# Geunwoo-Jeon/LarvaNet

Hardware: AMD Instinct MI355X
Metric: HR Mpixels/s (LarvaNet x4 multi-exit train step, 48x48 LR patches) (higher is better)
Workload: dtype f32; 1 GPU; LarvaNet x4 train_step_larva M4 B4,4,4,4 48ch, batch 16 of 3x48x48 -> 3x192x192 fp32 per GPU (BASELINE config 2); global_batch=16, parallelism=dp1, hip_graph=True

## Files before the change

larvanet_amd/csrc/conv3x3_mfma.hip:

```cpp
#include "larva_common.h"
#include "larva_bicubic.h"
#include <hip/hip_ext.h>
#include <cstdlib>
#include <type_traits>

#ifndef LARVA_DIAG
#define LARVA_DIAG 0
#endif
constexpr int kWgPerCu = 2;
constexpr int kOperandDepth = 2;


#ifndef LARVA_DIAG_ONLY48
#define LARVA_DIAG_ONLY48 0
#endif

namespace larva {

#if defined(LARVA_DIAG) && (LARVA_DIAG & 32)
__device__ unsigned long long* g_stamps = nullptr;
#if LARVA_DIAG & 512
constexpr int kDiagWgPerSlot = 256;
__device__ int g_slot_of_launch = 0;
__device__ __forceinline__ void stamp_slot(unsigned long long* area, int k) {
// ... 89 lines not shown
  static constexpr int CS = cout_stride(COUT);
  static constexpr int PS = G::PS;
  static constexpr int IN_PIECES = (kCh * PS + 255) / 256;
  static constexpr int IN_FLOATS = IN_PIECES * 256;
  static constexpr int IN_SLOTS_PER_PLANE = PS / 4;
  static constexpr int W_USED = 9 * kCh * CS;
  static constexpr int W_PIECES = (W_USED + 255) / 256;
  static constexpr int W_FLOATS = W_PIECES * 256;
  static constexpr int PIECES = IN_PIECES + W_PIECES;
  static constexpr int NPW = (PIECES + 3) / 4;
  static constexpr int STAGE_FLOATS = IN_FLOATS + W_FLOATS;
  static constexpr int STEPS = 9 * (kCh / 4);
  static constexpr int NST = 3;
  static constexpr int AHEAD = NST - 1;
  static constexpr size_t LDS_BYTES_DMA = NST * STAGE_FLOATS * sizeof(float);
  static constexpr bool LOADER = 2 * PIECES <= 63;
  static constexpr int THREADS_DMA = LOADER ? 320 : 256;
  static constexpr size_t LDS_BYTES_REG = 2 * STAGE_FLOATS * sizeof(float);
  static constexpr int RIN_SLOTS = kCh * G::HALO * (G::RS / 4);
  static constexpr int RIN_ITERS = (RIN_SLOTS + 255) / 256;
  static constexpr int RW_SLOTS = W_USED / 4;
  static constexpr int RW_ITERS = (RW_SLOTS + 255) / 256;
  static_assert(kCh * PS <= IN_FLOATS, "input planes must fit their pieces");
};

template <int COUT, typename G>
struct DmaPlan {
  unsigned voff[ConvCfg<COUT, G>::NPW];
};

template <int COUT, typename G, bool WEIGHTS>
__device__ __forceinline__ void make_plan(const ConvArgs& a, int wave, int lane, int y0, int x0,
                                          DmaPlan<COUT, G>& pl) {
  using C = ConvCfg<COUT, G>;
#pragma unroll
  for (int i = 0; i < C::NPW; ++i) {
    const int p = min(wave + 4 * i, C::PIECES - 1);
    const bool isw = p >= C::IN_PIECES;
    if constexpr (WEIGHTS) {
      if (4 * i + 3 < C::IN_PIECES) continue;
      const int ws = (p - C::IN_PIECES) * 64 + lane;
      if (isw) pl.voff[i] = (ws * 4 < C::W_USED) ? 16u * (unsigned)ws : kDmaZero;
    } else {
      if (4 * i >= C::IN_PIECES) continue;
      const int slot = p * 64 + lane;
      const int ci = slot / C::IN_SLOTS_PER_PLANE;
      const int rem = slot - ci * C::IN_SLOTS_PER_PLANE;
      const int r = rem / (G::RS / 4);
      const int q = rem - r * (G::RS / 4);
      const int gy = y0 - 1 + r, gx = x0 - 4 + 4 * q;
      const bool ok = ci < kCh && r < G::HALO && gy >= 0 && gy < a.H && gx >= 0 && gx < a.W;
      if (!isw) pl.voff[i] = ok ? 4u * (unsigned)((ci * a.H + gy) * a.pitch + gx) : kDmaZero;
    }
  }
}

struct ChunkSrc {
  i32x4 img;
  i32x4 wgt;
  const float* img_ptr;
  const float* wgt_ptr;
};

template <int COUT, typename G>
__device__ __forceinline__ ChunkSrc chunk_src(const ConvArgs& a, int chunk, int n, const float* src_override = nullptr) {
  using C = ConvCfg<COUT, G>;
  const int c0 = chunk * kCh;
  const int s_idx = div_by_magic(chunk, a.magic_cps);
  const int c_in_src = c0 - s_idx * a.cin_per_src;
  ChunkSrc cs;
  const float* src = src_override ? src_override : a.src[0];
  if (s_idx != 0) {
    asm volatile("" ::: "memory");
    src = a.src[s_idx];
  }
  cs.img_ptr = src + ((size_t)n * a.cin_per_src + c_in_src) * ((size_t)a.H * a.pitch);
  cs.wgt_ptr = a.wpk + (size_t)chunk * C::W_USED;
  cs.img = dma_rsrc(cs.img_ptr);
  cs.wgt = dma_rsrc(cs.wgt_ptr);
  return cs;
}

template <int COUT, typename G>
__device__ __forceinline__ void dma_piece(const DmaPlan<COUT, G>& pl, int i, int wave, const ChunkSrc& cs,
                                          unsigned stage_addr) {
  using C = ConvCfg<COUT, G>;
  const int p = min(wave + 4 * i, C::PIECES - 1);
  const bool isw = p >= C::IN_PIECES;
  i32x4 rsrc;
#pragma unroll
  for (int k = 0; k < 4; ++k) rsrc[k] = isw ? cs.wgt[k] : cs.img[k];
  lds_dma16_buf(rsrc, pl.voff[i], 0, stage_addr + 1024u * (unsigned)p);
}

template <int COUT, typename G>
struct LoaderPlan {
  unsigned voff[ConvCfg<COUT, G>::PIECES];
};

template <int COUT, typename G>
__device__ __forceinline__ void make_loader_plan(const ConvArgs& a, int lane, int y0, int x0, LoaderPlan<COUT, G>& pl) {
  using C = ConvCfg<COUT, G>;
#pragma unroll
  for (int p = 0; p < C::PIECES; ++p) {
    if (p < C::IN_PIECES) {
      const int slot = p * 64 + lane;
      const int ci = slot / C::IN_SLOTS_PER_PLANE;
      const int rem = slot - ci * C::IN_SLOTS_PER_PLANE;
      const int r = rem / (G::RS / 4);
      const int q = rem - r * (G::RS / 4);
      const int gy = y0 - 1 + r, gx = x0 - 4 + 4 * q;
      const bool ok = ci < kCh && r < G::HALO && gy >= 0 && gy < a.H && gx >= 0 && gx < a.W;
      pl.voff[p] = ok ? 4u * (unsigned)((ci * a.H + gy) * a.pitch + gx) : kDmaZero;
    } else {
      const int ws = (p - C::IN_PIECES) * 64 + lane;
      pl.voff[p] = (ws * 4 < C::W_USED) ? 16u * (unsigned)ws : kDmaZero;
    }
  }
}

template <int COUT, typename G>
__device__ __forceinline__ void run_loader(const ConvArgs& a, float* smem, int lane, int n, int y0, int x0) {
  using C = ConvCfg<COUT, G>;
  if constexpr ((LARVA_DIAG & 256) != 0) return;
  LoaderPlan<COUT, G> pl;
  make_loader_plan<COUT, G>(a, lane, y0, x0, pl);
  const int last = a.n_chunks - 1;
  int stage = 0;
  for (int chunk = 0; chunk <= last; ++chunk) {
    asm volatile("; LARVA_RING loader chunk_pieces=%1 ahead=%2\n\ts_waitcnt vmcnt(%0)\n\ts_barrier" ::"n"((C::AHEAD - 1) * C::PIECES), "n"(C::PIECES), "n"(C::AHEAD) : "memory");
    __builtin_amdgcn_sched_barrier(0);
    const int nstage = (stage + C::AHEAD) % C::NST;
    const unsigned dst = lds_addr_of(smem + nstage * C::STAGE_FLOATS);
    const ChunkSrc cs = chunk_src<COUT, G>(a, min(chunk + C::AHEAD, last), n);
#pragma unroll
    for (int p = 0; p < C::PIECES; ++p)
      lds_dma16_buf(p < C::IN_PIECES ? cs.img : cs.wgt, pl.voff[p], 0, dst + 1024u * (unsigned)p);
    stage = stage == C::NST - 1 ? 0 : stage + 1;
  }
  asm volatile("s_waitcnt vmcnt(0)" ::: "memory");
}

template <int COUT, typename G>
struct RegStaging {
  f32x4 in[ConvCfg<COUT, G>::RIN_ITERS];
  f32x4 w[ConvCfg<COUT, G>::RW_ITERS];
};

template <int COUT, typename G>
__device__ __forceinline__ void reg_load(const ConvArgs& a, const ChunkSrc& cs, int y0, int x0, int tid,
                                         RegStaging<COUT, G>& st) {
  using C = ConvCfg<COUT, G>;
  const size_t plane = (size_t)a.H * a.pitch;
#pragma unroll
  for (int i = 0; i < C::RIN_ITERS; ++i) {
    const int s = min(tid + i * 256, C::RIN_SLOTS - 1);
    const int ci = s / (G::HALO * (G::RS / 4));
    const int rem = s - ci * (G::HALO * (G::RS / 4));
    const int r = rem / (G::RS / 4);
    const int q = rem - r * (G::RS / 4);
    const int gy = y0 - 1 + r, gx = x0 - 4 + 4 * q;
    const bool row_ok = gy >= 0 && gy < a.H;
    const float* row = cs.img_ptr + (size_t)ci * plane + (size_t)min(max(gy, 0), a.H - 1) * a.pitch;
    f32x4 v;
#pragma unroll
    for (int e = 0; e < 4; ++e) {
// ... 35 lines not shown
template <int COUT, typename G, int NCT, int PG0, int NPG>
__device__ __forceinline__ void read_operands(const float* const (&a_base)[NCT], const float* b_base, int step,
                                              float (&av)[NCT], float (&bv)[NPG]) {
  using C = ConvCfg<COUT, G>;
  if constexpr ((LARVA_DIAG & 128) != 0) {
#pragma unroll
    for (int c = 0; c < NCT; ++c) av[c] = (float)step;
#pragma unroll
    for (int p = 0; p < NPG; ++p) bv[p] = (float)(step + p);
    return;
  }
  const int tap = step / (kCh / 4), kk = step % (kCh / 4);
  const int ky = tap / 3, kx = tap % 3;
#pragma unroll
  for (int c = 0; c < NCT; ++c) av[c] = a_base[c][(tap * kCh + kk * 4) * C::CS];
#pragma unroll
  for (int p = 0; p < NPG; ++p) {
    const int pg = PG0 + p, prow = pg / G::PC, pcol = pg % G::PC;
    bv[p] = b_base[kk * 4 * C::PS + (prow + ky) * G::RS + pcol * 16 + kx];
  }
}

template <int NMF, int NRD, int M>
__device__ __forceinline__ void shadow_groups() {
  if constexpr (M < NMF) {
    __builtin_amdgcn_sched_group_barrier(0x8, 1, 0);
    constexpr int share = (NRD + NMF - 1 - M) / NMF;
    if constexpr (share > 0) __builtin_amdgcn_sched_group_barrier(0x100, share, 0);
    shadow_groups<NMF, NRD, M + 1>();
  }
}

template <int COUT, typename G, int NCT, int PG0, int NPG, bool SWAP>
__device__ __forceinline__ void mfma_chunk(const float* stage, int ct0, int lane, f32x4 (&acc)[NCT][NPG],
                                           const float* wstage = nullptr) {
  using C = ConvCfg<COUT, G>;
  const int lr = lane & 15, lq = lane >> 4;
  const float* const wrows = wstage ? wstage : stage + C::IN_FLOATS;
  const float* a_base[NCT];
#pragma unroll
  for (int c = 0; c < NCT; ++c)
    a_base[c] = wrows + lq * C::CS + lr + (cout_swizzled(COUT) ? (((ct0 + c) ^ (lq & 1)) * 16) : (ct0 + c) * 16);
  const float* b_base = stage + lq * C::PS + lr + 3;
  constexpr int D = kOperandDepth;
  float av[D + 1][NCT], bv[D + 1][NPG];
#pragma unroll
  for (int d = 0; d < D; ++d)
    if (d < C::STEPS) read_operands<COUT, G, NCT, PG0, NPG>(a_base, b_base, d, av[d], bv[d]);
#pragma unroll
  for (int step = 0; step < C::STEPS; ++step) {
    __builtin_amdgcn_sched_barrier(0);
    if (step + D < C::STEPS)
      read_operands<COUT, G, NCT, PG0, NPG>(a_base, b_base, step + D, av[(step + D) % (D + 1)], bv[(step + D) % (D + 1)]);
    constexpr int NMF = NCT * NPG;
    constexpr int NRD = NCT + NPG;
#pragma unroll
    for (int m = 0; m < NMF; ++m) {
      const float wv = av[step % (D + 1)][m / NPG], xv = bv[step % (D + 1)][m % NPG];
      acc[m / NPG][m % NPG] = __builtin_amdgcn_mfma_f32_16x16x4f32(SWAP ? xv : wv, SWAP ? wv : xv, acc[m / NPG][m % NPG], 0, 0, 0);
    }
    shadow_groups<NMF, NRD, 0>();
    __builtin_amdgcn_sched_barrier(0);
  }
}

template <int KEEP, int PIECES, int AUX>
__device__ __forceinline__ void wait_and_barrier() {
  static_assert(KEEP == PIECES + AUX, "a ring wait keeps exactly the next chunk's pieces and the operand loads in flight");
  asm volatile("; LARVA_RING pieces=%1 aux=%2\n\ts_waitcnt vmcnt(%0)\n\ts_barrier" ::"n"(KEEP), "n"(PIECES), "n"(AUX) : "memory");
  __builtin_amdgcn_sched_barrier(0);
}

template <typename G>
__device__ __forceinline__ void decode_tile(const ConvArgs& a, int vb, int& n, int& y0, int& x0) {
  const int tile = xcd_remap(vb, a.nwg);
  const int t2 = div_by_magic(tile, a.magic_tx);
  const int tx = tile - t2 * a.tiles_x;
  n = div_by_magic(t2, a.magic_ty);
  const int ty = t2 - n * a.tiles_y;
  x0 = tx * G::COLS;
  y0 = ty * G::ROWS;
}

template <int COUT, typename G, bool VEC, int EPI, int NCT, int PG0, int NPG, bool PERSIST = false>
__device__ __forceinline__ void run_role(const ConvArgs& a, float* smem, int ct0, int wave, int n, int y0, int x0, int tid) {
  using C = ConvCfg<COUT, G>;
  static_assert(!VEC || C::LOADER, "the 16-byte path runs with a loader wave (2 * PIECES <= 63 for every instantiated shape)");
  static_assert(!PERSIST || VEC, "persistent tiles: the loader-wave path");
  const int lane = tid & 63;
  const int lr = lane & 15, lq = lane >> 4;
  float* const out_ptr = a.out;
  struct { int H, W, pitch, plain; } k = {a.H, a.W, a.pitch, a.plain_stores};
  asm volatile("" : "+s"(k.H), "+s"(k.W), "+s"(k.pitch), "+s"(k.plain));

  constexpr bool kShuffleEpi = (EPI == kEpiShuffle || EPI == kEpiShuffleBase || EPI == kEpiShuffleL1);
  constexpr bool kPixMajor = VEC && !kShuffleEpi;
  f32x4 bias[NCT];
#pragma unroll
  for (int c = 0; c < NCT; ++c) bias[c] = f32x4{0.f, 0.f, 0.f, 0.f};
  auto load_bias = [&]() {
    if (a.bias) {
#pragma unroll
      for (int c = 0; c < NCT; ++c)
#pragma unroll
        for (int r = 0; r < 4; ++r) bias[c][r] = a.bias[(ct0 + c) * 16 + (kPixMajor ? lr : lq * 4 + r)];
    }
  };

  constexpr int NAUX = (EPI == kEpiMask || EPI == kEpiRes1 || EPI == kEpiShuffleBase)
                           ? 1 : ((EPI == kEpiRes2 || EPI == kEpiShuffleL1) ? 2 : 0);
  f32x4 aux[NAUX > 0 ? NAUX : 1][NAUX > 0 ? NCT : 1][NAUX > 0 ? NPG : 1];
  constexpr int NU = NCT * NPG;
  constexpr int kEarlyPairs = PERSIST && COUT == 48 ? (NAUX * NU < 7 ? NAUX * NU : 7) : NAUX * NU;
  constexpr int kLatePart = 4, kEarlyAll = 5;
  auto load_aux = [&](int part = -1) {
#pragma unroll
    for (int c = 0; c < NCT; ++c)
#pragma unroll
      for (int p = 0; p < NPG; ++p) {
        const int pg = PG0 + p, prow = pg / G::PC, pcol = pg % G::PC;
        const int y = min(y0 + prow, a.H - 1), x = min(x0 + pcol * 16 + lr, a.W - 1);
        auto want = [&](int op) {
          const int q = op * NU + c * NPG + p;
          return part < 0 ? true : part == kLatePart ? q >= kEarlyPairs : q < kEarlyPairs;
        };
        if constexpr (kShuffleEpi) {
          const int HH = 4 * a.H, WW = 4 * a.W;
          const size_t idx = (((size_t)n * C::CT + (ct0 + c)) * HH + (4 * y + lq)) * WW + 4 * x;
          if (want(0)) aux[0][c][p] = *reinterpret_cast<const f32x4*>(a.base + idx);
          if constexpr (EPI == kEpiShuffleL1) {
            if (want(1)) aux[1][c][p] = *reinterpret_cast<const f32x4*>(a.truth + idx);
          }
        } else if constexpr (kPixMajor && (PERSIST || G::COLS == 16)) {
          const unsigned plane = (unsigned)a.H * (unsigned)a.pitch;
          const unsigned lane_off = 4u * ((unsigned)lr * plane + (unsigned)lq * 4u);
          const int soff = __builtin_amdgcn_readfirstlane(
              (int)(4u * ((unsigned)((ct0 + c) * 16) * plane + (unsigned)(y0 + prow) * (unsigned)a.pitch + (unsigned)(x0 + pcol * 16))));
          auto image = [&](const float* t) {
            const unsigned long long b = reinterpret_cast<unsigned long long>(t + (size_t)n * COUT * plane);
            const unsigned lo = (unsigned)__builtin_amdgcn_readfirstlane((int)(unsigned)b);
            const unsigned hi = (unsigned)__builtin_amdgcn_readfirstlane((int)(unsigned)(b >> 32));
            return __builtin_amdgcn_make_buffer_rsrc(reinterpret_cast<void*>(((unsigned long long)hi << 32) | lo), 0,
                                                     (int)(COUT * plane * 4u), 0x00020000);
          };
          if constexpr (EPI == kEpiMask) {
            if (want(0)) aux[0][c][p] = __builtin_bit_cast(f32x4, __builtin_amdgcn_raw_buffer_load_b128(image(a.mask), lane_off, soff, 0));
          }
          if constexpr (EPI == kEpiRes1 || EPI == kEpiRes2) {
            if (want(0)) aux[0][c][p] = __builtin_bit_cast(f32x4, __builtin_amdgcn_raw_buffer_load_b128(image(a.res0), lane_off, soff, 0));
          }
          if constexpr (EPI == kEpiRes2) {
            if (want(1)) aux[1][c][p] = __builtin_bit_cast(f32x4, __builtin_amdgcn_raw_buffer_load_b128(image(a.res1), lane_off, soff, 0));
          }
        } else if constexpr (kPixMajor) {
          const size_t plane = (size_t)a.H * a.pitch;
          const int xb = min(x0 + pcol * 16 + lq * 4, a.pitch - 4);
          const size_t idx = ((size_t)n * COUT + (ct0 + c) * 16 + lr) * plane + (size_t)y * a.pitch + xb;
          if constexpr (EPI == kEpiMask) {
            if (want(0)) aux[0][c][p] = *reinterpret_cast<const f32x4*>(a.mask + idx);
          }
          if constexpr (EPI == kEpiRes1 || EPI == kEpiRes2) {
            if (want(0)) aux[0][c][p] = *reinterpret_cast<const f32x4*>(a.res0 + idx);
          }
          if constexpr (EPI == kEpiRes2) {
            if (want(1)) aux[1][c][p] = *reinterpret_cast<const f32x4*>(a.res1 + idx);
          }
        } else {
          const size_t plane = (size_t)a.H * a.pitch;
          const size_t idx0 = ((size_t)n * COUT + (ct0 + c) * 16 + lq * 4) * plane + (size_t)y * a.pitch + x;
#pragma unroll
          for (int r = 0; r < 4; ++r) {
            if constexpr (EPI == kEpiMask) aux[0][c][p][r] = a.mask[idx0 + r * plane];
            if constexpr (EPI == kEpiRes1 || EPI == kEpiRes2) aux[0][c][p][r] = a.res0[idx0 + r * plane];
            if constexpr (EPI == kEpiRes2) aux[1][c][p][r] = a.res1[idx0 + r * plane];
          }
        }
      }
  };
  constexpr bool kAuxLate = VEC && !kShuffleEpi && !(LARVA_DIAG & 6) && NAUX > 0 && !PERSIST;
  constexpr int kAuxLoads = kAuxLate ? NAUX * NCT * NPG : 0;
  auto load_early = [&]() {
    load_bias();
    if constexpr (NAUX > 0 && !kAuxLate && !(LARVA_DIAG & 4)) load_aux();
  };
  int pstage = 0;
  for (int vb = blockIdx.x;; vb += gridDim.x) {
  if constexpr (PERSIST) {
    if (vb >= a.nwg) break;
    decode_tile<G>(a, vb, n, y0, x0);
  }
  if constexpr (!VEC || (LARVA_DIAG & 2)) load_early();

  f32x4 acc[NCT][NPG];
#pragma unroll
  for (int c = 0; c < NCT; ++c)
#pragma unroll
    for (int p = 0; p < NPG; ++p) acc[c][p] = f32x4{0.f, 0.f, 0.f, 0.f};

  if constexpr (PERSIST) {
    load_bias();
    const int my_chunk = a.n_chunks >= 4 ? (wave & 3) : 0;
    __builtin_amdgcn_sched_barrier(0);
    for (int chunk = 0; chunk < a.n_chunks; ++chunk) {
      asm volatile("s_barrier" ::: "memory");
      __builtin_amdgcn_sched_barrier(0);
      if constexpr (NAUX > 0) {
        if (chunk == my_chunk) load_aux(kEarlyAll);
        __builtin_amdgcn_sched_barrier(0);
      }
      mfma_chunk<COUT, G, NCT, PG0, NPG, kPixMajor>(smem + pstage * C::STAGE_FLOATS, ct0, lane, acc);
      pstage = pstage == C::NST - 1 ? 0 : pstage + 1;
    }
    asm volatile("s_waitcnt vmcnt(0)" ::: "memory");
    __builtin_amdgcn_sched_barrier(0);
    if constexpr (kEarlyPairs < NAUX * NU) {
      load_aux(kLatePart);
      __builtin_amdgcn_sched_barrier(0);
    }
  } else if constexpr (VEC) {
    DmaPlan<COUT, G> pl;
    const int last = a.n_chunks - 1;
    if constexpr (!(LARVA_DIAG & 2)) {
      const ChunkSrc cs0 = chunk_src<COUT, G>(a, 0, n);
      const unsigned st0 = lds_addr_of(smem), st1 = lds_addr_of(smem + C::STAGE_FLOATS);
      stamp(6);
      make_plan<COUT, G, true>(a, wave, lane, y0, x0, pl);
#pragma unroll
      for (int i = 0; i < C::NPW; ++i)
        if (wave + 4 * i >= C::IN_PIECES) dma_piece<COUT, G>(pl, i, wave, cs0, st0);
      __builtin_amdgcn_sched_barrier(0);
      stamp(7);
      load_early();
      stamp(14);
      make_plan<COUT, G, false>(a, wave, lane, y0, x0, pl);
#pragma unroll
      for (int i = 0; i < C::NPW; ++i)
        if (wave + 4 * i < C::IN_PIECES) dma_piece<COUT, G>(pl, i, wave, cs0, st0);
      stamp(15);
      const ChunkSrc cs1 = chunk_src<COUT, G>(a, min(1, last), n);
#pragma unroll
      for (int i = 0; i < C::NPW; ++i) dma_piece<COUT, G>(pl, i, wave, cs1, st1);
      if constexpr (kAuxLate) {
        __builtin_amdgcn_sched_barrier(0);
        load_aux();
        __builtin_amdgcn_sched_barrier(0);
      }
    }
    stamp(1);
    int stage = 0;
    for (int chunk = 0; chunk <= last; ++chunk) {
      if constexpr ((LARVA_DIAG & 256) != 0) {
      } else if (chunk == 0) wait_and_barrier<((LARVA_DIAG & 2) ? 0 : C::NPW) + kAuxLoads, ((LARVA_DIAG & 2) ? 0 : C::NPW), kAuxLoads>();
      else wait_and_barrier<kAuxLoads, 0, kAuxLoads>();
      if (chunk == 0) stamp(2);
      stamp(8 + (chunk < 7 ? chunk : 7));
      if constexpr (!(LARVA_DIAG & 1)) mfma_chunk<COUT, G, NCT, PG0, NPG, kPixMajor>(smem + stage * C::STAGE_FLOATS, ct0, lane, acc);
      stage = stage == C::NST - 1 ? 0 : stage + 1;
    }
    asm volatile("s_waitcnt vmcnt(0)" ::: "memory");
    stamp(3);
  } else {
    RegStaging<COUT, G> st;
    if constexpr (!(LARVA_DIAG & 2)) {
      reg_load<COUT, G>(a, chunk_src<COUT, G>(a, 0, n), y0, x0, tid, st);
      reg_store<COUT, G>(smem, tid, st);
    }
    __syncthreads();
    for (int chunk = 0; chunk < a.n_chunks; ++chunk) {
      float* cur = smem + (chunk & 1) * C::STAGE_FLOATS;
      float* nxt = smem + ((chunk & 1) ^ 1) * C::STAGE_FLOATS;
      const bool more = chunk + 1 < a.n_chunks;
      if constexpr (!(LARVA_DIAG & 2)) {
        if (more) reg_load<COUT, G>(a, chunk_src<COUT, G>(a, chunk + 1, n), y0, x0, tid, st);
      }
      if constexpr (!(LARVA_DIAG & 1)) mfma_chunk<COUT, G, NCT, PG0, NPG, kPixMajor>(cur, ct0, lane, acc);
      if constexpr (!(LARVA_DIAG & 2)) {
        if (more) reg_store<COUT, G>(nxt, tid, st);
      }
      __syncthreads();
    }
  }

  if constexpr ((LARVA_DIAG & 4) != 0) {
#pragma unroll
    for (int c = 0; c < NCT; ++c)
#pragma unroll
      for (int p = 0; p < NPG; ++p) asm volatile("" ::"v"(acc[c][p]));
    return;
  }

  if constexpr (EPI == kEpiShuffleL1) {
    const int HH = 4 * k.H, WW = 4 * k.W;
    const size_t plane = (size_t)k.H * k.pitch;
    const float g = a.gval;
    float s = 0.f;
#pragma unroll
    for (int c = 0; c < NCT; ++c)
#pragma unroll
      for (int p = 0; p < NPG; ++p) {
        const int pg = PG0 + p, prow = pg / G::PC, pcol = pg % G::PC;
        const int y = y0 + prow, x = x0 + pcol * 16 + lr;
        const f32x4 v = (acc[c][p] + bias[c]) + aux[0][c][p];
        if (y < k.H && x < k.W) {
          if (out_ptr) {
            const size_t idx = (((size_t)n * C::CT + (ct0 + c)) * HH + (4 * y + lq)) * WW + 4 * x;
            __builtin_nontemporal_store(v, reinterpret_cast<f32x4*>(out_ptr + idx));
          }
          const f32x4 d = v - aux[1][c][p];
          s += fabsf(d[0]) + fabsf(d[1]) + fabsf(d[2]) + fabsf(d[3]);
          const size_t idx0 = ((size_t)n * COUT + (ct0 + c) * 16 + lq * 4) * plane + (size_t)y * k.pitch + x;
#pragma unroll
          for (int r = 0; r < 4; ++r)
            __builtin_nontemporal_store(d[r] > 0.f ? g : (d[r] < 0.f ? -g : 0.f), &a.grad[idx0 + r * plane]);
        }
      }
#pragma unroll
    for (int o = 32; o > 0; o >>= 1) s += __shfl_xor(s, o);
    if (lane == 0) a.partial[4 * blockIdx.x + wave] = s;
  } else if constexpr (EPI == kEpiShuffle || EPI == kEpiShuffleBase) {
    const int HH = 4 * k.H, WW = 4 * k.W;
#pragma unroll
    for (int c = 0; c < NCT; ++c)
#pragma unroll
      for (int p = 0; p < NPG; ++p) {
        const int pg = PG0 + p, prow = pg / G::PC, pcol = pg % G::PC;
        const int y = y0 + prow, x = x0 + pcol * 16 + lr;
        const size_t idx = (((size_t)n * C::CT + (ct0 + c)) * HH + (4 * y + lq)) * WW + 4 * x;
        f32x4 v = acc[c][p] + bias[c];
        if constexpr (EPI == kEpiShuffleBase) v += aux[0][c][p];
        if (y < k.H && x < k.W) __builtin_nontemporal_store(v, reinterpret_cast<f32x4*>(out_ptr + idx));
      }
  } else if constexpr (kPixMajor) {
    const size_t plane = (size_t)k.H * k.pitch;
    auto store_all = [&](auto plain_tag, auto interior_tag) {
      constexpr bool kPlain = decltype(plain_tag)::value;
      constexpr bool kInterior = decltype(interior_tag)::value;
#pragma unroll
      for (int c = 0; c < NCT; ++c)
#pragma unroll
        for (int p = 0; p < NPG; ++p) {
          const int pg = PG0 + p, prow = pg / G::PC, pcol = pg % G::PC;
          const int y = y0 + prow, xb = x0 + pcol * 16 + lq * 4;
          const size_t idx = ((size_t)n * COUT + (ct0 + c) * 16 + lr) * plane + (size_t)y * k.pitch + xb;
          f32x4 v = acc[c][p] + bias[c];
          if (kInterior || (y < k.H && xb < k.pitch)) {
#pragma unroll
            for (int r = 0; r < 4; ++r) {
              float o = v[r];
              if constexpr (EPI == kEpiRelu) o = fmaxf(o, 0.f);
              if constexpr (EPI == kEpiMask) o = (aux[0][c][p][r] > 0.f) ? o : 0.f;
              if constexpr (EPI == kEpiRes1 || EPI == kEpiRes2) o += aux[0][c][p][r];
              if constexpr (EPI == kEpiRes2) o += aux[1][c][p][r];
              v[r] = (kInterior || xb + r < k.W) ? o : 0.f;
            }
            if constexpr (kPlain) *reinterpret_cast<f32x4*>(out_ptr + idx) = v;
            else __builtin_nontemporal_store(v, reinterpret_cast<f32x4*>(out_ptr + idx));
          }
        }
    };
    constexpr bool kFastPath = EPI == kEpiPlain || EPI == kEpiRelu || EPI == kEpiRes1;
    const bool interior = kFastPath && y0 + G::ROWS <= k.H && x0 + G::COLS <= k.W;
    auto store_policy = [&](auto plain_tag) {
      if constexpr (kFastPath) {
        if (interior) {
          store_all(plain_tag, std::true_type{});
          return;
        }
      }
      store_all(plain_tag, std::false_type{});
    };
    if constexpr ((LARVA_DIAG & 16) != 0) {
      store_policy(std::true_type{});
    } else if constexpr (G::COLS == 16) {
      if (k.plain) store_policy(std::true_type{});
      else store_policy(std::false_type{});
    } else {
      store_policy(std::false_type{});
    }
  } else {
    const size_t plane = (size_t)k.H * k.pitch;
#pragma unroll
    for (int c = 0; c < NCT; ++c)
#pragma unroll
      for (int p = 0; p < NPG; ++p) {
        const int pg = PG0 + p, prow = pg / G::PC, pcol = pg % G::PC;
        const int y = y0 + prow, x = x0 + pcol * 16 + lr;
        const size_t idx0 = ((size_t)n * COUT + (ct0 + c) * 16 + lq * 4) * plane + (size_t)y * k.pitch + x;
        const f32x4 v = acc[c][p] + bias[c];
        if (y < k.H && x < k.pitch) {
          const bool real = x < k.W;
#pragma unroll
          for (int r = 0; r < 4; ++r) {
            float o = v[r];
            if constexpr (EPI == kEpiRelu) o = fmaxf(o, 0.f);
            if constexpr (EPI == kEpiMask) o = (aux[0][c][p][r] > 0.f) ? o : 0.f;
            if constexpr (EPI == kEpiRes1 || EPI == kEpiRes2) o += aux[0][c][p][r];
            if constexpr (EPI == kEpiRes2) o += aux[1][c][p][r];
            o = real ? o : 0.f;
            if constexpr ((LARVA_DIAG & 16) != 0) out_ptr[idx0 + r * plane] = o;
            else __builtin_nontemporal_store(o, &out_ptr[idx0 + r * plane]);
          }
        }
      }
  }
#if LARVA_DIAG & 32
  stamp(4);
  asm volatile("s_waitcnt vmcnt(0)" ::: "memory");
  stamp(5);
#endif
  if constexpr (!PERSIST) break;
  }
}

__device__ __forceinline__ void fetch_args(const ConvArgs& a) {
  asm volatile("" ::"s"(a.src[0]), "s"(a.wpk), "s"(a.bias), "s"(a.out), "s"(a.cin_per_src), "s"(a.n_chunks), "s"(a.N),
               "s"(a.H), "s"(a.W), "s"(a.pitch), "s"(a.tiles_x), "s"(a.tiles_y), "s"(a.magic_tx), "s"(a.magic_ty),
               "s"(a.magic_cps), "s"(a.nwg), "s"(a.tile_tab), "s"(a.plain_stores), "s"(a.tab_n),
               "s"(a.tab16[0]), "s"(a.tab16[16]));
}

template <int COUT, bool VEC, int EPI, typename G = GeoWide>
__device__ __forceinline__ void conv_tile(const ConvArgs& a, float* smem) {
  if constexpr ((LARVA_DIAG & 8) != 0) return;
  stamp(0);
  fetch_args(a);
  const int tile = xcd_remap(blockIdx.x, a.nwg);
  const int t2 = div_by_magic(tile, a.magic_tx);
  const int tx = tile - t2 * a.tiles_x;
  const int n = div_by_magic(t2, a.magic_ty);
  const int ty = t2 - n * a.tiles_y;
  const int x0 = tx * G::COLS, y0 = ty * G::ROWS;
  const int tid = threadIdx.x;
  const int wave = __builtin_amdgcn_readfirstlane(tid >> 6);
  __builtin_amdgcn_s_setprio(1);

  if constexpr (VEC) {
    if (wave == 4) {
      if constexpr (!(LARVA_DIAG & 2)) run_loader<COUT, G>(a, smem, tid & 63, n, y0, x0);
      return;
    }
  }
  if constexpr (G::ROWS == 4) {
    static_assert(VEC && (COUT == 48 || COUT == 32), "4 x 48 tiles: the 16-byte path at 48 / 32 channels");
    if constexpr (COUT == 48) {
      if (wave < 3) run_role<COUT, G, VEC, EPI, 1, 0, 9>(a, smem, wave, wave, n, y0, x0, tid);
      else run_role<COUT, G, VEC, EPI, 3, 9, 3>(a, smem, 0, wave, n, y0, x0, tid);
    } else {
      if (wave < 2) run_role<COUT, G, VEC, EPI, 1, 0, 6>(a, smem, wave, wave, n, y0, x0, tid);
      else run_role<COUT, G, VEC, EPI, 1, 6, 6>(a, smem, wave - 2, wave, n, y0, x0, tid);
    }
  } else if constexpr (COUT == 48) {
    if (wave < 3) run_role<COUT, G, VEC, EPI, 1, 0, 7>(a, smem, wave, wave, n, y0, x0, tid);
    else run_role<COUT, G, VEC, EPI, 3, 7, 2>(a, smem, 0, wave, n, y0, x0, tid);
  } else if constexpr (COUT == 32) {
    if (wave < 2) run_role<COUT, G, VEC, EPI, 1, 0, 5>(a, smem, wave, wave, n, y0, x0, tid);
    else run_role<COUT, G, VEC, EPI, 1, 5, 4>(a, smem, wave - 2, wave, n, y0, x0, tid);
  } else {
    static_assert(COUT == 64, "unsupported channel count");
    run_role<COUT, G, VEC, EPI, 1, 0, 9>(a, smem, wave, wave, n, y0, x0, tid);
  }
}

template <int COUT, bool VEC, int EPI>
__global__ __launch_bounds__(VEC ? ConvCfg<COUT>::THREADS_DMA : 256, VEC ? kWgPerCu : 1) void conv3x3_mfma_kernel(ConvArgs a) {
  extern __shared__ __attribute__((aligned(16))) float smem[];
  conv_tile<COUT, VEC, EPI>(a, smem);
}

template <int COUT, int EPI>
__global__ __launch_bounds__((ConvCfg<COUT, GeoWide4>::THREADS_DMA), kWgPerCu) void conv3x3_mfma_rows4_kernel(ConvArgs a) {
  extern __shared__ __attribute__((aligned(16))) float smem[];
  conv_tile<COUT, true, EPI, GeoWide4>(a, smem);
}
static_assert(2 * ConvCfg<48, GeoWide4>::LDS_BYTES_DMA <= 160 * 1024, "two 4 x 48 workgroups per CU");

template <int COUT, typename G>
__device__ __forceinline__ void run_loader_persist(const ConvArgs& a, float* smem, int lane) {
  using C = ConvCfg<COUT, G>;
  static_assert(C::NST == 3 && 2 * C::PIECES <= 63, "three stages, two chunks in flight");
  LoaderPlan<COUT, G> pl;
  int vb_i = blockIdx.x, n_i, y0, x0, c_i = 0, s_i = 0;
  decode_tile<G>(a, vb_i, n_i, y0, x0);
  make_loader_plan<COUT, G>(a, lane, y0, x0, pl);
  bool more = true;
  auto issue = [&]() {
    const ChunkSrc cs = chunk_src<COUT, G>(a, c_i, n_i);
    const unsigned dst = lds_addr_of(smem + s_i * C::STAGE_FLOATS);
#pragma unroll
    for (int p = 0; p < C::PIECES; ++p)
      lds_dma16_buf(p < C::IN_PIECES ? cs.img : cs.wgt, pl.voff[p], 0, dst + 1024u * (unsigned)p);
    s_i = s_i == C::NST - 1 ? 0 : s_i + 1;
    if (++c_i == a.n_chunks) {
      c_i = 0;
      vb_i += gridDim.x;
      more = vb_i < a.nwg;
      if (more) {
        decode_tile<G>(a, vb_i, n_i, y0, x0);
        make_loader_plan<COUT, G>(a, lane, y0, x0, pl);
      }
    }
  };
  int ahead = 0;
  issue();
  ++ahead;
  if (more) {
    issue();
    ++ahead;
  }
  while (ahead > 0) {
    if (ahead == 2) asm volatile("s_waitcnt vmcnt(%0)" ::"n"(C::PIECES) : "memory");
    else asm volatile("s_waitcnt vmcnt(0)" ::: "memory");
    asm volatile("s_barrier" ::: "memory");
    __builtin_amdgcn_sched_barrier(0);
    --ahead;
    if (more) {
      issue();
      ++ahead;
    }
  }
}

template <int COUT, int EPI>
__global__ __launch_bounds__((ConvCfg<COUT>::THREADS_DMA), kWgPerCu) void conv3x3_mfma_persist_kernel(ConvArgs a) {
  extern __shared__ __attribute__((aligned(16))) float smem[];
  using G = GeoWide;
  stamp(0);
  fetch_args(a);
  const int tid = threadIdx.x;
  const int wave = __builtin_amdgcn_readfirstlane(tid >> 6);
  __builtin_amdgcn_s_setprio(1);
  if (wave == 4) {
    run_loader_persist<COUT, G>(a, smem, tid & 63);
    return;
  }
  if constexpr (COUT == 48) {
    if (wave < 3) run_role<COUT, G, true, EPI, 1, 0, 7, true>(a, smem, wave, wave, 0, 0, 0, tid);
    else run_role<COUT, G, true, EPI, 3, 7, 2, true>(a, smem, 0, wave, 0, 0, 0, tid);
  } else if constexpr (COUT == 32) {
    if (wave < 2) run_role<COUT, G, true, EPI, 1, 0, 5, true>(a, smem, wave, wave, 0, 0, 0, tid);
    else run_role<COUT, G, true, EPI, 1, 5, 4, true>(a, smem, wave - 2, wave, 0, 0, 0, tid);
  } else {
    static_assert(COUT == 64, "unsupported channel count");
    run_role<COUT, G, true, EPI, 1, 0, 9, true>(a, smem, wave, wave, 0, 0, 0, tid);
  }
}

template <int COUT, int EPI, typename G>
__device__ __forceinline__ void strip_roles(const ConvArgs& a, float* smem, int wave, int n, int y0, int x0, int tid) {
  static_assert(ConvCfg<COUT, G>::LOADER, "the strip kernel is launched with a loader wave");
  static_assert(COUT == 48 || COUT == 32 || COUT == 64, "strip tiles: 32, 48 or 64 output channels");
  if (wave == 4) {
    run_loader<COUT, G>(a, smem, tid & 63, n, y0, x0);
    return;
  }
  if constexpr (COUT == 64) {
    run_role<COUT, G, true, EPI, 1, 0, G::ROWS>(a, smem, wave, wave, n, y0, x0, tid);
  } else if constexpr (COUT == 48) {
    if (wave < 3) run_role<COUT, G, true, EPI, 1, 0, G::ROWS - 1>(a, smem, wave, wave, n, y0, x0, tid);
    else run_role<COUT, G, true, EPI, 3, G::ROWS - 1, 1>(a, smem, 0, wave, n, y0, x0, tid);
  } else if constexpr (G::ROWS == 5) {
    if (wave < 2) run_role<COUT, G, true, EPI, 1, 0, 3>(a, smem, wave, wave, n, y0, x0, tid);
    else if (wave == 2) run_role<COUT, G, true, EPI, 2, 3, 1>(a, smem, 0, wave, n, y0, x0, tid);
    else run_role<COUT, G, true, EPI, 2, 4, 1>(a, smem, 0, wave, n, y0, x0, tid);
  } else {
    if (wave < 2) run_role<COUT, G, true, EPI, 1, 0, 2>(a, smem, wave, wave, n, y0, x0, tid);
    else run_role<COUT, G, true, EPI, 1, 2, 2>(a, smem, wave - 2, wave, n, y0, x0, tid);
  }
}

template <int COUT, int EPI>
__global__ __launch_bounds__(320, kWgPerCu) void conv3x3_mfma_strip_kernel(ConvArgs a) {
  extern __shared__ __attribute__((aligned(16))) float smem[];
  stamp(0);
  fetch_args(a);
  const int tile = xcd_remap(blockIdx.x, a.nwg);
  const int n = div_by_magic(tile, a.magic_tx);
  const int slot = tile - n * a.tiles_x;
  unsigned e;
  if (a.tab_n) {
    const unsigned pair = (unsigned)a.tab16[slot >> 1];
    const unsigned h = (slot & 1) ? pair >> 16 : pair & 0xffffu;
    e = (h & 0xffu) | (((h >> 8) & 0x7fu) << 16) | ((h >> 15) << 31);
  } else {
    e = a.tile_tab[slot];
  }
  const int y0 = (int)(e & 0xfffu), x0 = (int)((e >> 12) & 0xfffu);
  const int tid = threadIdx.x;
  const int wave = __builtin_amdgcn_readfirstlane(tid >> 6);
  __builtin_amdgcn_s_setprio(1);
  if (e >> 31) strip_roles<COUT, EPI, GeoS5>(a, smem, wave, n, y0, x0, tid);
  else strip_roles<COUT, EPI, GeoS4>(a, smem, wave, n, y0, x0, tid);
}
template <int COUT>
constexpr size_t kStripLdsBytes = ConvCfg<COUT, GeoS5>::LDS_BYTES_DMA > ConvCfg<COUT, GeoS4>::LDS_BYTES_DMA ? ConvCfg<COUT, GeoS5>::LDS_BYTES_DMA
                                                                                                            : ConvCfg<COUT, GeoS4>::LDS_BYTES_DMA;
static_assert(kWgPerCu * kStripLdsBytes<48> <= 160 * 1024 && kWgPerCu * kStripLdsBytes<64> <= 160 * 1024, "strip workgroups per CU");

constexpr int kMaxConvJobs = 4;
struct ConvBatch {
  ConvArgs job[kMaxConvJobs];
};

template <int COUT, int EPI>
__global__ __launch_bounds__(ConvCfg<COUT>::THREADS_DMA, kWgPerCu) void conv3x3_mfma_batch_kernel(ConvBatch b) {
  extern __shared__ __attribute__((aligned(16))) float smem[];
  conv_tile<COUT, true, EPI>(b.job[blockIdx.y], smem);
}

constexpr int kMaxPackJobs = 64;

struct PackJob {
  const float* w;
  float* fwd;
  float* bwd;
  int cout, cin, w_cin_total, w_cin_off;
};

struct PackBatch {
  PackJob job[kMaxPackJobs];
};

__host__ __device__ constexpr int packed_floats(int cout, int cin) {
  return (cin / kCh) * 9 * kCh * cout_stride(cout);
}

constexpr int kPackTileCols = 64;
constexpr int kPackLd = kPackTileCols + 1;
constexpr int kPackTileFloats = 9 * kCh * kPackLd;

__host__ __device__ constexpr int pack_slots(int cout, int cin) { return cin / kCh + cout / kCh; }

__device__ __forceinline__ void pack_block(const PackJob& j, int slot, float* __restrict__ tile) {
  const int nfc = j.cin / kCh;
  const bool fwd = slot < nfc;
  const int chunk = fwd ? slot : slot - nfc;
  float* __restrict__ out = fwd ? j.fwd : j.bwd;
  if ((!fwd && chunk >= j.cout / kCh) || !out) return;
  const int cols = fwd ? j.cout : j.cin;
  const int cs = cout_stride(cols);
  const int tid = threadIdx.x;
  out += (size_t)chunk * 72 * cs;
  for (int c0 = 0; c0 < cs; c0 += kPackTileCols) {
    const int ncol = min(kPackTileCols, cols - c0);
    if (fwd) {
      for (int idx = tid; idx < ncol * 72; idx += 256) {
        const int c = idx / 72, r = idx - c * 72, k = r / 9, tap = r - k * 9;
        const int cin_abs = j.w_cin_off + chunk * kCh + k;
        tile[(tap * kCh + k) * kPackLd + c] =
            cin_abs < j.w_cin_total ? j.w[((size_t)(c0 + c) * j.w_cin_total + cin_abs) * 9 + tap] : 0.f;
      }
    } else {
      const int row = ncol * 9;
      for (int idx = tid; idx < kCh * row; idx += 256) {
        const int k = idx / row, rem = idx - k * row, c = rem / 9, tap = rem - c * 9;
        tile[((8 - tap) * kCh + k) * kPackLd + c] =
            j.w_cin_off + c0 + c < j.w_cin_total
                ? j.w[((size_t)(chunk * kCh + k) * j.w_cin_total + j.w_cin_off + c0) * 9 + rem] : 0.f;
      }
    }
    __syncthreads();
    const int wcols = min(kPackTileCols, cs - c0);
    const bool swz = cout_swizzled(cols);
    for (int idx = tid; idx < 72 * wcols; idx += 256) {
      const int r = idx / wcols, c = idx - r * wcols;
      const int col = swz ? ((c0 + c) ^ ((r & 1) << 4)) : c0 + c;
      out[r * cs + col] = c < ncol ? tile[r * kPackLd + c] : 0.f;
    }
    __syncthreads();
  }
}

__global__ __launch_bounds__(256) void pack_weights_batch_kernel(PackBatch b) {
  __shared__ float tile[kPackTileFloats];
  pack_block(b.job[blockIdx.y], blockIdx.x, tile);
}

constexpr int kPrologueBlocks = 192;
constexpr int kProloguePadSlices = 2, kPrologueBicSlices = 8;
struct PrologueArgs {
  PackBatch packs;
  int npack, slots;
  const float* x;
  float* x16;
  float* base;
  int N, C, H, W;
};

__global__ __launch_bounds__(256) void step_prologue_kernel(PrologueArgs a) {
  __shared__ float tile[kPackTileFloats];
  int blk = blockIdx.x;
  if (blk < a.npack * a.slots) {
    const int job = blk / a.slots;
    pack_block(a.packs.job[job], blk - job * a.slots, tile);
    return;
  }
  blk -= a.npack * a.slots;
  constexpr int nthr = kPrologueBlocks * 256;
  const int slice = blk / kPrologueBlocks, tid = (blk - slice * kPrologueBlocks) * 256 + threadIdx.x;
  const int nbic = a.base ? kPrologueBicSlices : 0;
  if (slice < nbic) {
    bicubic4_body(a.x, a.base, a.N * a.C, a.H, a.W, (long long)slice * nthr + tid, (long long)nthr * kPrologueBicSlices);
  } else {
    const int plane = a.H * a.W, per_img = a.C * plane, total = a.N * per_img;
    for (int i = (slice - nbic) * nthr + tid; i < total; i += nthr * kProloguePadSlices) {
      const int n = i / per_img, r = i - n * per_img;
      a.x16[(size_t)n * 16 * plane + r] = a.x[i];
    }
  }
}

struct LaunchTiming {
  hipEvent_t start, stop;
};

template <auto Kernel, typename Args>
static hipError_t launch(dim3 grid, dim3 block, size_t lds, hipStream_t stream, const LaunchTiming* tm, const Args& a) {
  static PerDeviceOnce lds_set;
  if (const hipError_t e = ensure_dynamic_lds(lds_set, reinterpret_cast<const void*>(Kernel), lds); e != hipSuccess) return e;
  if (tm)
    hipExtLaunchKernelGGL(Kernel, grid, block, lds, stream, tm->start, tm->stop, 0, a);
  else
    hipLaunchKernelGGL(Kernel, grid, block, lds, stream, a);
  return hipGetLastError();
}

template <int... E>
struct EpiSet {
  static constexpr bool has(int epi) { return ((epi == E) || ...); }
};
using EpiAll = EpiSet<kEpiPlain, kEpiRelu, kEpiMask, kEpiRes1, kEpiRes2, kEpiShuffle, kEpiShuffleBase>;
using EpiBatch48 = EpiSet<kEpiPlain, kEpiRelu, kEpiMask, kEpiRes1, kEpiRes2, kEpiShuffle, kEpiShuffleBase, kEpiShuffleL1>;
using EpiInference = EpiSet<kEpiPlain, kEpiRelu, kEpiRes1, kEpiRes2, kEpiShuffle, kEpiShuffleBase>;
using EpiRows4 = EpiInference;
using EpiPersist = EpiInference;

template <int... E, typename F>
static hipError_t with_epi(EpiSet<E...>, int epi, hipError_t absent, F&& f) {
  hipError_t r = absent;
  (void)((epi == E && (r = f(std::integral_constant<int, E>{}), true)) || ...);
  return r;
}

template <typename F>
static hipError_t with_cout(int cout, hipError_t absent, F&& f) {
  switch (cout) {
#if !LARVA_DIAG_ONLY48
    case 32: return f(std::integral_constant<int, 32>{});
    case 64: return f(std::integral_constant<int, 64>{});
#endif
    case 48: return f(std::integral_constant<int, 48>{});
    default: return absent;
  }
}

static int conv_slots() { return kWgPerCu * device_cu_count(); }

template <int COUT>
static hipError_t launch_conv(const ConvArgs& a, bool vec, int epi, hipStream_t stream, const LaunchTiming* tm) {
  using C = ConvCfg<COUT>;
  const dim3 grid(a.N * a.tiles_x * a.tiles_y);
  return with_epi(EpiAll{}, epi, hipErrorInvalidValue, [&](auto e) {
    constexpr int EPI = decltype(e)::value;
    if (vec)
      return launch<conv3x3_mfma_kernel<COUT, true, EPI>>(grid, dim3(C::THREADS_DMA), C::LDS_BYTES_DMA, stream, tm, a);
    return launch<conv3x3_mfma_kernel<COUT, false, EPI>>(grid, dim3(256), C::LDS_BYTES_REG, stream, tm, a);
  });
}

template <int COUT>
static hipError_t launch_rows4(const ConvArgs& a, int epi, hipStream_t stream, const LaunchTiming* tm) {
  using C = ConvCfg<COUT, GeoWide4>;
  return with_epi(EpiRows4{}, epi, hipErrorNotSupported, [&](auto e) {
    return launch<conv3x3_mfma_rows4_kernel<COUT, decltype(e)::value>>(dim3(a.nwg), dim3(C::THREADS_DMA), C::LDS_BYTES_DMA,
                                                                      stream, tm, a);
  });
}

template <int COUT>
static hipError_t launch_persist(const ConvArgs& a, int epi, hipStream_t stream, const LaunchTiming* tm) {
  using C = ConvCfg<COUT>;
  if ((long long)COUT * a.H * a.pitch * 4 >= (1ll << 31)) return hipErrorNotSupported;
  const int grid = a.nwg < conv_slots() ? a.nwg : conv_slots();
  return with_epi(EpiPersist{}, epi, hipErrorNotSupported, [&](auto e) {
    return launch<conv3x3_mfma_persist_kernel<COUT, decltype(e)::value>>(dim3(grid), dim3(C::THREADS_DMA), C::LDS_BYTES_DMA,
                                                                        stream, tm, a);
  });
}

template <int COUT>
static hipError_t launch_batch(const ConvBatch& b, int njobs, int epi, hipStream_t stream) {
  using C = ConvCfg<COUT>;
  using Set = std::conditional_t<COUT == 48, EpiBatch48, EpiAll>;
  const ConvArgs& a = b.job[0];
  return with_epi(Set{}, epi, epi == kEpiShuffleL1 ? hipErrorNotSupported : hipErrorInvalidValue, [&](auto e) {
    return launch<conv3x3_mfma_batch_kernel<COUT, decltype(e)::value>>(dim3(a.N * a.tiles_x * a.tiles_y, njobs),
                                                                      dim3(C::THREADS_DMA), C::LDS_BYTES_DMA, stream,
                                                                      nullptr, b);
  });
}

template <int COUT>
static hipError_t launch_strip(const ConvArgs& a, int epi, hipStream_t stream, const LaunchTiming* tm) {
  return with_epi(EpiAll{}, epi, hipErrorInvalidValue, [&](auto e) {
    return launch<conv3x3_mfma_strip_kernel<COUT, decltype(e)::value>>(dim3(a.nwg), dim3(320), kStripLdsBytes<COUT>, stream,
                                                                      tm, a);
  });
}

}

using namespace larva;

extern "C" {

long long larva_packed_weight_floats(int cout, int cin) { return (long long)packed_floats(cout, cin); }

static int fill_pack_jobs(PackBatch& b, const float* const* w, float* const* wpk_fwd, float* const* wpk_bwd,
                          const int* cout, const int* cin, const int* w_cin_total, const int* w_cin_off, int njobs) {
  int slots = 0;
  for (int i = 0; i < njobs; ++i) {
    if (!w[i] || cout[i] % kCh || cin[i] % kCh || cout[i] <= 0 || cin[i] <= 0) return -1;
    b.job[i] = PackJob{w[i], wpk_fwd[i], wpk_bwd[i], cout[i], cin[i], w_cin_total[i], w_cin_off[i]};
    const int n = pack_slots(cout[i], cin[i]);
    slots = n > slots ? n : slots;
  }
  return slots;
}

int larva_pack_weights_batch(const float* const* w, float* const* wpk_fwd, float* const* wpk_bwd,
                             const int* cout, const int* cin, const int* w_cin_total,
                             const int* w_cin_off, int njobs, void* stream) {
  if (njobs < 1 || njobs > kMaxPackJobs) return (int)hipErrorInvalidValue;
  PackBatch b{};
  const int slots = fill_pack_jobs(b, w, wpk_fwd, wpk_bwd, cout, cin, w_cin_total, w_cin_off, njobs);
  if (slots < 1) return (int)hipErrorInvalidValue;
  hipLaunchKernelGGL(pack_weights_batch_kernel, dim3(slots, njobs), dim3(256), 0, (hipStream_t)stream, b);
  return (int)hipGetLastError();
}

int larva_step_prologue(const float* const* w, float* const* wpk_fwd, float* const* wpk_bwd, const int* cout,
                        const int* cin, const int* w_cin_total, const int* w_cin_off, int njobs, const float* x,
                        float* x16, float* base, int N, int C, int H, int W, void* stream) {
  if (njobs < 0 || njobs > kMaxPackJobs || !x || N <= 0 || C <= 0 || C > 16 || H <= 0 || W <= 0)
    return (int)hipErrorInvalidValue;
  if ((long long)N * 16 * H * W >= (1ll << 31)) return (int)hipErrorInvalidValue;
  if (base && (reinterpret_cast<uintptr_t>(base) & 15)) return (int)hipErrorInvalidValue;
  PrologueArgs a{};
  a.slots = njobs ? fill_pack_jobs(a.packs, w, wpk_fwd, wpk_bwd, cout, cin, w_cin_total, w_cin_off, njobs) : 0;
  if (a.slots < 0) return (int)hipErrorInvalidValue;
  a.npack = njobs;
  a.x = x; a.x16 = x16; a.base = base;
  a.N = N; a.C = C; a.H = H; a.W = W;
  if (!x16 && base) return (int)hipErrorInvalidValue;
  const int blocks = njobs * a.slots + kPrologueBlocks * ((base ? kPrologueBicSlices : 0) + (x16 ? kProloguePadSlices : 0));
  if (blocks == 0) return 0;
  hipLaunchKernelGGL(step_prologue_kernel, dim3(blocks), dim3(256), 0, (hipStream_t)stream, a);
  return (int)hipGetLastError();
}

int larva_pack_weights(const float* w, float* wpk_fwd, float* wpk_bwd, int cout, int cin,
                       int w_cin_total, int w_cin_off, void* stream) {
  return larva_pack_weights_batch(&w, &wpk_fwd, &wpk_bwd, &cout, &cin, &w_cin_total, &w_cin_off, 1, stream);
}

#if LARVA_DIAG & 512
static int g_diag_next_slot = -1, g_diag_slot_cap = 0;
static unsigned long long* g_diag_host_base = nullptr;
static int diag_take_slot() {
  if (g_diag_next_slot < 0 || g_diag_next_slot >= g_diag_slot_cap) return -1;
  return g_diag_next_slot++;
}
int larva_diag_arm_slots(int first, int cap) {
  const int was = g_diag_next_slot;
  g_diag_next_slot = first;
  g_diag_slot_cap = cap;
  return was;
// ... 277 lines not shown
```

Before: 361.9 HR Mpixels/s.

## Walk batched 48-channel conv jobs with a persistent-tile kernel

```diff
diff --git a/larvanet_amd/csrc/conv3x3_mfma.hip b/larvanet_amd/csrc/conv3x3_mfma.hip
--- a/larvanet_amd/csrc/conv3x3_mfma.hip
+++ b/larvanet_amd/csrc/conv3x3_mfma.hip
@@ -195,6 +195,25 @@
 }
 
 template <int COUT, typename G>
+__device__ __forceinline__ ChunkSrc chunk_src_of(const ConvArgs& a, const ConvArgs& pa, int chunk, int n, const float* src0,
+                                                 const float* wpk) {
+  using C = ConvCfg<COUT, G>;
+  const int s_idx = div_by_magic(chunk, a.magic_cps);
+  const int c_in_src = chunk * kCh - s_idx * a.cin_per_src;
+  const float* src = src0;
+  if (s_idx != 0) {
+    asm volatile("" ::: "memory");
+    src = pa.src[s_idx];
+  }
+  ChunkSrc cs;
+  cs.img_ptr = src + ((size_t)n * a.cin_per_src + c_in_src) * ((size_t)a.H * a.pitch);
+  cs.wgt_ptr = wpk + (size_t)chunk * C::W_USED;
+  cs.img = dma_rsrc(cs.img_ptr);
+  cs.wgt = dma_rsrc(cs.wgt_ptr);
+  return cs;
+}
+
+template <int COUT, typename G>
 __device__ __forceinline__ void dma_piece(const DmaPlan<COUT, G>& pl, int i, int wave, const ChunkSrc& cs,
                                           unsigned stage_addr) {
   using C = ConvCfg<COUT, G>;
@@ -396,14 +415,17 @@
   y0 = ty * G::ROWS;
 }
 
-template <int COUT, typename G, bool VEC, int EPI, int NCT, int PG0, int NPG, bool PERSIST = false>
-__device__ __forceinline__ void run_role(const ConvArgs& a, float* smem, int ct0, int wave, int n, int y0, int x0, int tid) {
+template <int COUT, typename G, bool VEC, int EPI, int NCT, int PG0, int NPG, bool PERSIST = false, bool WALK = false>
+__device__ __forceinline__ void run_role(const ConvArgs& a, float* smem, int ct0, int wave, int n, int y0, int x0, int tid,
+                                         const ConvArgs* jobs = nullptr, int items = 0) {
   using C = ConvCfg<COUT, G>;
   static_assert(!VEC || C::LOADER, "the 16-byte path runs with a loader wave (2 * PIECES <= 63 for every instantiated shape)");
   static_assert(!PERSIST || VEC, "persistent tiles: the loader-wave path");
+  static_assert(!WALK || PERSIST, "a batch is walked on persistent tiles");
   const int lane = tid & 63;
   const int lr = lane & 15, lq = lane >> 4;
-  float* const out_ptr = a.out;
+  float* out_ptr = a.out;
+  const ConvArgs* ap = &a;
   struct { int H, W, pitch, plain; } k = {a.H, a.W, a.pitch, a.plain_stores};
   asm volatile("" : "+s"(k.H), "+s"(k.W), "+s"(k.pitch), "+s"(k.plain));
 
@@ -413,11 +435,11 @@
 #pragma unroll
   for (int c = 0; c < NCT; ++c) bias[c] = f32x4{0.f, 0.f, 0.f, 0.f};
   auto load_bias = [&]() {
-    if (a.bias) {
+    if (ap->bias) {
 #pragma unroll
       for (int c = 0; c < NCT; ++c)
 #pragma unroll
-        for (int r = 0; r < 4; ++r) bias[c][r] = a.bias[(ct0 + c) * 16 + (kPixMajor ? lr : lq * 4 + r)];
+        for (int r = 0; r < 4; ++r) bias[c][r] = ap->bias[(ct0 + c) * 16 + (kPixMajor ? lr : lq * 4 + r)];
     }
   };
 
@@ -441,9 +463,9 @@
         if constexpr (kShuffleEpi) {
           const int HH = 4 * a.H, WW = 4 * a.W;
           const size_t idx = (((size_t)n * C::CT + (ct0 + c)) * HH + (4 * y + lq)) * WW + 4 * x;
-          if (want(0)) aux[0][c][p] = *reinterpret_cast<const f32x4*>(a.base + idx);
+          if (want(0)) aux[0][c][p] = *reinterpret_cast<const f32x4*>(ap->base + idx);
           if constexpr (EPI == kEpiShuffleL1) {
-            if (want(1)) aux[1][c][p] = *reinterpret_cast<const f32x4*>(a.truth + idx);
+            if (want(1)) aux[1][c][p] = *reinterpret_cast<const f32x4*>(ap->truth + idx);
           }
         } else if constexpr (kPixMajor && (PERSIST || G::COLS == 16)) {
           const unsigned plane = (unsigned)a.H * (unsigned)a.pitch;
@@ -458,35 +480,35 @@
                                                      (int)(COUT * plane * 4u), 0x00020000);
           };
           if constexpr (EPI == kEpiMask) {
-            if (want(0)) aux[0][c][p] = __builtin_bit_cast(f32x4, __builtin_amdgcn_raw_buffer_load_b128(image(a.mask), lane_off, soff, 0));
+            if (want(0)) aux[0][c][p] = __builtin_bit_cast(f32x4, __builtin_amdgcn_raw_buffer_load_b128(image(ap->mask), lane_off, soff, 0));
           }
           if constexpr (EPI == kEpiRes1 || EPI == kEpiRes2) {
-            if (want(0)) aux[0][c][p] = __builtin_bit_cast(f32x4, __builtin_amdgcn_raw_buffer_load_b128(image(a.res0), lane_off, soff, 0));
+            if (want(0)) aux[0][c][p] = __builtin_bit_cast(f32x4, __builtin_amdgcn_raw_buffer_load_b128(image(ap->res0), lane_off, soff, 0));
           }
           if constexpr (EPI == kEpiRes2) {
-            if (want(1)) aux[1][c][p] = __builtin_bit_cast(f32x4, __builtin_amdgcn_raw_buffer_load_b128(image(a.res1), lane_off, soff, 0));
+            if (want(1)) aux[1][c][p] = __builtin_bit_cast(f32x4, __builtin_amdgcn_raw_buffer_load_b128(image(ap->res1), lane_off, soff, 0));
           }
         } else if constexpr (kPixMajor) {
           const size_t plane = (size_t)a.H * a.pitch;
           const int xb = min(x0 + pcol * 16 + lq * 4, a.pitch - 4);
           const size_t idx = ((size_t)n * COUT + (ct0 + c) * 16 + lr) * plane + (size_t)y * a.pitch + xb;
           if constexpr (EPI == kEpiMask) {
-            if (want(0)) aux[0][c][p] = *reinterpret_cast<const f32x4*>(a.mask + idx);
+            if (want(0)) aux[0][c][p] = *reinterpret_cast<const f32x4*>(ap->mask + idx);
           }
           if constexpr (EPI == kEpiRes1 || EPI == kEpiRes2) {
-            if (want(0)) aux[0][c][p] = *reinterpret_cast<const f32x4*>(a.res0 + idx);
+            if (want(0)) aux[0][c][p] = *reinterpret_cast<const f32x4*>(ap->res0 + idx);
           }
           if constexpr (EPI == kEpiRes2) {
-            if (want(1)) aux[1][c][p] = *reinterpret_cast<const f32x4*>(a.res1 + idx);
+            if (want(1)) aux[1][c][p] = *reinterpret_cast<const f32x4*>(ap->res1 + idx);
           }
         } else {
           const size_t plane = (size_t)a.H * a.pitch;
           const size_t idx0 = ((size_t)n * COUT + (ct0 + c) * 16 + lq * 4) * plane + (size_t)y * a.pitch + x;
 #pragma unroll
           for (int r = 0; r < 4; ++r) {
-            if constexpr (EPI == kEpiMask) aux[0][c][p][r] = a.mask[idx0 + r * plane];
-            if constexpr (EPI == kEpiRes1 || EPI == kEpiRes2) aux[0][c][p][r] = a.res0[idx0 + r * plane];
-            if constexpr (EPI == kEpiRes2) aux[1][c][p][r] = a.res1[idx0 + r * plane];
+            if constexpr (EPI == kEpiMask) aux[0][c][p][r] = ap->mask[idx0 + r * plane];
+            if constexpr (EPI == kEpiRes1 || EPI == kEpiRes2) aux[0][c][p][r] = ap->res0[idx0 + r * plane];
+            if constexpr (EPI == kEpiRes2) aux[1][c][p][r] = ap->res1[idx0 + r * plane];
           }
         }
       }
@@ -499,7 +521,16 @@
   };
   int pstage = 0;
   for (int vb = blockIdx.x;; vb += gridDim.x) {
-  if constexpr (PERSIST) {
+  int pidx = vb;
+  if constexpr (WALK) {
+    if (vb >= items) break;
+    const int job = (vb >= a.nwg ? 1 : 0) + (vb >= 2 * a.nwg ? 1 : 0) + (vb >= 3 * a.nwg ? 1 : 0);
+    pidx = vb - job * a.nwg;
+    const ConvArgs& aj = jobs[job];
+    ap = &aj;
+    out_ptr = aj.out;
+    decode_tile<G>(a, pidx, n, y0, x0);
+  } else if constexpr (PERSIST) {
     if (vb >= a.nwg) break;
     decode_tile<G>(a, vb, n, y0, x0);
   }
@@ -625,12 +656,12 @@
           const size_t idx0 = ((size_t)n * COUT + (ct0 + c) * 16 + lq * 4) * plane + (size_t)y * k.pitch + x;
 #pragma unroll
           for (int r = 0; r < 4; ++r)
-            __builtin_nontemporal_store(d[r] > 0.f ? g : (d[r] < 0.f ? -g : 0.f), &a.grad[idx0 + r * plane]);
+            __builtin_nontemporal_store(d[r] > 0.f ? g : (d[r] < 0.f ? -g : 0.f), &ap->grad[idx0 + r * plane]);
         }
       }
 #pragma unroll
     for (int o = 32; o > 0; o >>= 1) s += __shfl_xor(s, o);
-    if (lane == 0) a.partial[4 * blockIdx.x + wave] = s;
+    if (lane == 0) ap->partial[4 * pidx + wave] = s;
   } else if constexpr (EPI == kEpiShuffle || EPI == kEpiShuffleBase) {
     const int HH = 4 * k.H, WW = 4 * k.W;
 #pragma unroll
@@ -788,17 +819,33 @@
 }
 static_assert(2 * ConvCfg<48, GeoWide4>::LDS_BYTES_DMA <= 160 * 1024, "two 4 x 48 workgroups per CU");
 
-template <int COUT, typename G>
-__device__ __forceinline__ void run_loader_persist(const ConvArgs& a, float* smem, int lane) {
+template <int COUT, typename G, bool WALK = false>
+__device__ __forceinline__ void run_loader_persist(const ConvArgs& a, float* smem, int lane, const ConvArgs* jobs = nullptr,
+                                                   int items = 0) {
   using C = ConvCfg<COUT, G>;
   static_assert(C::NST == 3 && 2 * C::PIECES <= 63, "three stages, two chunks in flight");
   LoaderPlan<COUT, G> pl;
   int vb_i = blockIdx.x, n_i, y0, x0, c_i = 0, s_i = 0;
-  decode_tile<G>(a, vb_i, n_i, y0, x0);
-  make_loader_plan<COUT, G>(a, lane, y0, x0, pl);
+  const int total = WALK ? items : a.nwg;
+  int job_i = 0;
+  const float *src_i = nullptr, *wpk_i = nullptr;
+  auto enter_item = [&]() {
+    int tile = vb_i;
+    if constexpr (WALK) {
+      job_i = (vb_i >= a.nwg ? 1 : 0) + (vb_i >= 2 * a.nwg ? 1 : 0) + (vb_i >= 3 * a.nwg ? 1 : 0);
+      tile = vb_i - job_i * a.nwg;
+      src_i = jobs[job_i].src[0];
+      wpk_i = jobs[job_i].wpk;
+    }
+    decode_tile<G>(a, tile, n_i, y0, x0);
+    make_loader_plan<COUT, G>(a, lane, y0, x0, pl);
+  };
+  enter_item();
   bool more = true;
   auto issue = [&]() {
-    const ChunkSrc cs = chunk_src<COUT, G>(a, c_i, n_i);
+    ChunkSrc cs;
+    if constexpr (WALK) cs = chunk_src_of<COUT, G>(a, jobs[job_i], c_i, n_i, src_i, wpk_i);
+    else cs = chunk_src<COUT, G>(a, c_i, n_i);
     const unsigned dst = lds_addr_of(smem + s_i * C::STAGE_FLOATS);
 #pragma unroll
     for (int p = 0; p < C::PIECES; ++p)
@@ -807,11 +854,8 @@
     if (++c_i == a.n_chunks) {
       c_i = 0;
       vb_i += gridDim.x;
-      more = vb_i < a.nwg;
-      if (more) {
-        decode_tile<G>(a, vb_i, n_i, y0, x0);
-        make_loader_plan<COUT, G>(a, lane, y0, x0, pl);
-      }
+      more = vb_i < total;
+      if (more) enter_item();
     }
   };
   int ahead = 0;
@@ -913,12 +957,33 @@
 constexpr int kMaxConvJobs = 4;
 struct ConvBatch {
   ConvArgs job[kMaxConvJobs];
+  int njobs;
 };
 
 template <int COUT, int EPI>
 __global__ __launch_bounds__(ConvCfg<COUT>::THREADS_DMA, kWgPerCu) void conv3x3_mfma_batch_kernel(ConvBatch b) {
   extern __shared__ __attribute__((aligned(16))) float smem[];
   conv_tile<COUT, true, EPI>(b.job[blockIdx.y], smem);
+}
+
+template <int COUT, int EPI>
+__global__ __launch_bounds__(ConvCfg<COUT>::THREADS_DMA, kWgPerCu) void conv3x3_mfma_batch_persist_kernel(ConvBatch b) {
+  extern __shared__ __attribute__((aligned(16))) float smem[];
+  using G = GeoWide;
+  static_assert(COUT == 48, "the walking batch kernel: 48 output channels");
+  const ConvArgs& a = b.job[0];
+  stamp(0);
+  fetch_args(a);
+  const int items = b.njobs * a.nwg;
+  const int tid = threadIdx.x;
+  const int wave = __builtin_amdgcn_readfirstlane(tid >> 6);
+  __builtin_amdgcn_s_setprio(1);
+  if (wave == 4) {
+    run_loader_persist<COUT, G, true>(a, smem, tid & 63, b.job, items);
+    return;
+  }
+  if (wave < 3) run_role<COUT, G, true, EPI, 1, 0, 7, true, true>(a, smem, wave, wave, 0, 0, 0, tid, b.job, items);
+  else run_role<COUT, G, true, EPI, 3, 7, 2, true, true>(a, smem, 0, wave, 0, 0, 0, tid, b.job, items);
 }
 
 constexpr int kMaxPackJobs = 64;
@@ -1046,7 +1111,8 @@
 using EpiBatch48 = EpiSet<kEpiPlain, kEpiRelu, kEpiMask, kEpiRes1, kEpiRes2, kEpiShuffle, kEpiShuffleBase, kEpiShuffleL1>;
 using EpiInference = EpiSet<kEpiPlain, kEpiRelu, kEpiRes1, kEpiRes2, kEpiShuffle, kEpiShuffleBase>;
 using EpiRows4 = EpiInference;
-using EpiPersist = EpiInference;
+using EpiPersist = EpiSet<kEpiPlain, kEpiRelu, kEpiMask, kEpiRes1, kEpiRes2, kEpiShuffle, kEpiShuffleBase>;
+using EpiBatchPersist = EpiSet<kEpiMask, kEpiShuffleL1>;
 
 template <int... E, typename F>
 static hipError_t with_epi(EpiSet<E...>, int epi, hipError_t absent, F&& f) {
@@ -1106,6 +1172,19 @@
   using C = ConvCfg<COUT>;
   using Set = std::conditional_t<COUT == 48, EpiBatch48, EpiAll>;
   const ConvArgs& a = b.job[0];
+  if constexpr (COUT == 48) {
+    const char* pe = getenv("LARVA_PERSIST");
+    const bool persist_on = !(pe && pe[0] == '0');
+    const long long items = (long long)njobs * a.nwg;
+    if (persist_on && items > conv_slots() && EpiBatchPersist::has(epi) && (long long)COUT * a.H * a.pitch * 4 < (1ll << 31)) {
+      ConvBatch w = b;
+      w.njobs = njobs;
+      return with_epi(EpiBatchPersist{}, epi, hipErrorInvalidValue, [&](auto e) {
+        return launch<conv3x3_mfma_batch_persist_kernel<COUT, decltype(e)::value>>(dim3(conv_slots()), dim3(C::THREADS_DMA),
+                                                                                C::LDS_BYTES_DMA, stream, nullptr, w);
+      });
+    }
+  }
   return with_epi(Set{}, epi, epi == kEpiShuffleL1 ? hipErrorNotSupported : hipErrorInvalidValue, [&](auto e) {
     return launch<conv3x3_mfma_batch_kernel<COUT, decltype(e)::value>>(dim3(a.N * a.tiles_x * a.tiles_y, njobs),
                                                                       dim3(C::THREADS_DMA), C::LDS_BYTES_DMA, stream,
```

Result: no change. 363.7 HR Mpixels/s, median of 6 (+0.5%).
